# serizard/DeltaKD

Measured on NVIDIA B200. Metric: distill-loss fwd+bwd samples/s, higher is better.
Workload: dtype bf16

## Files before the change

### deltakd_b200/csrc/logit_kd.cu

```cuda
#include <stdlib.h>

#include "common.cuh"

#ifndef DKD_LOGIT_STAMP
#define DKD_LOGIT_STAMP(point, dep) ((void)0)
#endif
#ifndef DKD_LOGIT_FOLD_STAMP
#define DKD_LOGIT_FOLD_STAMP(point, dep) ((void)0)
#endif

namespace dkd {
namespace {

constexpr int kThreads = 128;

__device__ __forceinline__ float fexp(float x) {
  float y;
  asm("ex2.approx.ftz.f32 %0, %1;" : "=f"(y) : "f"(x * 1.4426950408889634f));
  return y;
}
__device__ __forceinline__ float fexp2(float x, float k2, float m2) {
  float y;
  asm("ex2.approx.ftz.f32 %0, %1;" : "=f"(y) : "f"(fmaf(x, k2, -m2)));
  return y;
}

__device__ __forceinline__ float2 ex2_2(float2 x) {
  float2 y;
  asm("ex2.approx.ftz.f32 %0, %1;" : "=f"(y.x) : "f"(x.x));
  asm("ex2.approx.ftz.f32 %0, %1;" : "=f"(y.y) : "f"(x.y));
  return y;
}

struct LogitKdParams {
  const void* z;
  const void* zk;
  const void* zt;
  const void* y;
  void* gz;
  void* gzk;
  float* loss_out;
  float* row_base;
  float* row_kd;
  unsigned int* ticket;
  int64_t B, C;
  int label_kind, kd_kind;
  float smoothing, alpha, tau;
  const float* mix_lam;
};

constexpr int kRuntimeMode = -2;
constexpr float kL2e = 1.4426950408889634f;
template <typename T, int VEC, int NV, int THREADS = kThreads, int LK = kRuntimeMode, int KK = kRuntimeMode,
          bool PACK2 = (THREADS == kThreads), typename Publish>
__device__ __forceinline__ void logit_row(const LogitKdParams& p, int64_t row, const T* z, const T* zk, const T* zt, const T* y,
                                          T* gz_row, T* gzk_row, float* scratch, int* s_arg, float* s_argv, float& base_out,
                                          float& kd_out, Publish&& publish) {
  const int64_t C = p.C;
  const int label_kind = LK == kRuntimeMode ? p.label_kind : LK;
  const int kd_kind = KK == kRuntimeMode ? p.kd_kind : KK;
  const int tid = THREADS == 32 ? (int)(threadIdx.x & 31) : (int)threadIdx.x;
  const int64_t label = label_kind == 1 ? reinterpret_cast<const int64_t*>(p.y)[row] : -1;
  const bool mixing = label_kind == 1 && p.mix_lam != nullptr;
  const int64_t label2 = mixing ? reinterpret_cast<const int64_t*>(p.y)[p.B - 1 - row] : -1;
  const float lam = mixing ? __ldg(p.mix_lam) : 1.f;
  const float invT = kd_kind == 1 ? 1.f / p.tau : 1.f;

  constexpr int NVR = NV > 0 ? NV : 1;
  float rz[NVR][VEC], rk[NVR][VEC], rt[NVR][VEC], ry[NVR][VEC];
  const int nchunk = (int)((C + (int64_t)THREADS * VEC - 1) / ((int64_t)THREADS * VEC));

  auto col_of = [&](int it) -> int64_t { return ((int64_t)it * THREADS + tid) * VEC; };
  const T* any = label_kind >= 0 ? z : zk;
  const T* lz = label_kind >= 0 ? z : any;
  const T* lzk = kd_kind ? zk : any;
  const T* lzt = kd_kind ? zt : any;
  const T* ly = label_kind == 0 ? y : any;
  auto load4 = [&](int it, float (&a)[VEC], float (&b)[VEC], float (&c)[VEC], float (&d)[VEC]) {
    const int64_t col0 = col_of(it);
    const int64_t col = col0 < C ? col0 : 0;
    Vec<T, VEC>::load(lz + col, a);
    Vec<T, VEC>::load(lzk + col, b);
    Vec<T, VEC>::load(lzt + col, c);
    Vec<T, VEC>::load(ly + col, d);
    if (label_kind < 0) {
#pragma unroll
      for (int v = 0; v < VEC; ++v) a[v] = 0.f;
    }
  };

  float mx[3] = {-INFINITY, -INFINITY, -INFINITY};
  float best = -INFINITY;
  int64_t best_i = INT64_MAX;
  auto pass1 = [&](int it, float (&a)[VEC], float (&b)[VEC], float (&c)[VEC]) {
    const int64_t col = col_of(it);
    if (col < C) {
#pragma unroll
      for (int v = 0; v < VEC; ++v) {
        mx[0] = fmaxf(mx[0], a[v]);
        if (kd_kind) {
          mx[1] = fmaxf(mx[1], b[v]);
          mx[2] = fmaxf(mx[2], c[v]);
          if (kd_kind == 2 && c[v] > best) { best = c[v]; best_i = col + v; }
        }
      }
    }
  };
  if constexpr (NV > 0) {
#pragma unroll
    for (int it = 0; it < NV; ++it)
      if (it < nchunk) load4(it, rz[it], rk[it], rt[it], ry[it]);
#pragma unroll
    for (int it = 0; it < NV; ++it)
      if (it < nchunk) pass1(it, rz[it], rk[it], rt[it]);
  } else {
    for (int it = 0; it < nchunk; ++it) {
      load4(it, rz[0], rk[0], rt[0], ry[0]);
      pass1(it, rz[0], rk[0], rt[0]);
    }
  }
  DKD_LOGIT_STAMP(1, mx[0]);
  block_max<3, THREADS>(mx, scratch);
  DKD_LOGIT_STAMP(2, mx[0]);
  mx[1] *= invT;
  mx[2] *= invT;
  int64_t tgt = label;
  int64_t hard_idx = -1;
  if (kd_kind == 2) {
    float bv = best;
    long long bi = (long long)best_i;
#pragma unroll
    for (int o = 16; o > 0; o >>= 1) {
      float ov = __shfl_xor_sync(0xffffffffu, bv, o);
      long long oi = __shfl_xor_sync(0xffffffffu, bi, o);
      if (ov > bv || (ov == bv && oi < bi)) { bv = ov; bi = oi; }
    }
    if constexpr (THREADS > 32) {
      __syncthreads();
      if ((threadIdx.x & 31) == 0) { s_argv[threadIdx.x >> 5] = bv; s_arg[threadIdx.x >> 5] = (int)bi; }
      __syncthreads();
      bv = s_argv[0]; bi = s_arg[0];
#pragma unroll
      for (int w = 1; w < THREADS / 32; ++w) {
        if (s_argv[w] > bv || (s_argv[w] == bv && s_arg[w] < bi)) { bv = s_argv[w]; bi = s_arg[w]; }
      }
    }
    hard_idx = bi;
  }
  (void)tgt;

  float st8[8] = {0.f, 0.f, 0.f, 0.f, 0.f, 0.f, 0.f, 0.f};
  float (&s)[4] = *reinterpret_cast<float(*)[4]>(&st8[0]);
  float (&t)[4] = *reinterpret_cast<float(*)[4]>(&st8[4]);
  constexpr bool PACKED = NV > 0 && VEC % 2 == 0 && PACK2;
  float2 S2[4], T2[2];
#pragma unroll
  for (int k = 0; k < 4; ++k) S2[k] = make_float2(0.f, 0.f);
  T2[0] = T2[1] = make_float2(0.f, 0.f);
  auto pass2 = [&](int it, float (&a)[VEC], float (&b)[VEC], float (&c)[VEC], float (&d)[VEC]) {
    const int64_t col = col_of(it);
    if (col < C) {
      if constexpr (PACKED) {
        const float2 kz = splat2(kL2e), nm0 = splat2(-mx[0] * kL2e);
        const float2 kt = splat2(invT * kL2e), nm1 = splat2(-mx[1] * kL2e), nm2 = splat2(-mx[2] * kL2e);
#pragma unroll
        for (int v = 0; v < VEC; v += 2) {
          const float2 A = make_float2(a[v], a[v + 1]);
          const float2 ea = ex2_2(fma2(A, kz, nm0));
          S2[0] = add2(S2[0], ea);
          if (label_kind == 0) {
            const float2 D = make_float2(d[v], d[v + 1]);
            T2[0] = add2(T2[0], D);
            T2[1] = fma2(D, A, T2[1]);
          } else {
            T2[1] = add2(T2[1], A);
            if (col + v == label) t[2] = a[v];
            if (col + v + 1 == label) t[2] = a[v + 1];
            if (col + v == label2) t[0] = a[v];
            if (col + v + 1 == label2) t[0] = a[v + 1];
          }
          a[v] = ea.x; a[v + 1] = ea.y;
          if (kd_kind == 1) {
            const float2 Bv = make_float2(b[v], b[v + 1]), Cv = make_float2(c[v], c[v + 1]);
            const float2 eb = ex2_2(fma2(Cv, kt, nm2)), es = ex2_2(fma2(Bv, kt, nm1));
            S2[1] = add2(S2[1], es);
            S2[2] = add2(S2[2], eb);
            S2[3] = fma2(eb, sub2(Cv, Bv), S2[3]);
            b[v] = es.x; b[v + 1] = es.y;
            c[v] = eb.x; c[v + 1] = eb.y;
          } else if (kd_kind == 2) {
            const float2 Bv = make_float2(b[v], b[v + 1]);
            const float2 es = ex2_2(fma2(Bv, kz, nm1));
            S2[1] = add2(S2[1], es);
            if (col + v == hard_idx) t[3] = b[v];
            if (col + v + 1 == hard_idx) t[3] = b[v + 1];
            b[v] = es.x; b[v + 1] = es.y;
          }
        }
        return;
      }
#pragma unroll
      for (int v = 0; v < VEC; ++v) {
        const float ea = fexp2(a[v], kL2e, mx[0] * kL2e);
        s[0] += ea;
        if (label_kind == 0) { t[0] += d[v]; t[1] += d[v] * a[v]; }
        else { t[1] += a[v]; if (col + v == label) t[2] = a[v]; if (col + v == label2) t[0] = a[v]; }
        if (NV > 0) a[v] = ea;
        if (kd_kind == 1) {
          const float eb = fexp2(c[v], invT * kL2e, mx[2] * kL2e), es = fexp2(b[v], invT * kL2e, mx[1] * kL2e);
          s[1] += es;
          s[2] += eb;
          s[3] = fmaf(eb, c[v] - b[v], s[3]);
          if (NV > 0) { b[v] = es; c[v] = eb; }
        } else if (kd_kind == 2) {
          const float es = fexp2(b[v], kL2e, mx[1] * kL2e);
          s[1] += es;
          if (col + v == hard_idx) t[3] = b[v];
          if (NV > 0) b[v] = es;
        }
      }
    }
  };
  if constexpr (NV > 0) {
#pragma unroll
    for (int it = 0; it < NV; ++it) if (it < nchunk) pass2(it, rz[it], rk[it], rt[it], ry[it]);
  } else {
    for (int it = 0; it < nchunk; ++it) {
      load4(it, rz[0], rk[0], rt[0], ry[0]);
      pass2(it, rz[0], rk[0], rt[0], ry[0]);
    }
  }
  if constexpr (PACKED) {
#pragma unroll
    for (int k = 0; k < 4; ++k) s[k] = S2[k].x + S2[k].y;
    if (label_kind == 0) t[0] = T2[0].x + T2[0].y;
    t[1] = T2[1].x + T2[1].y;
  }
  block_sum<8, THREADS>(st8, scratch);
  DKD_LOGIT_STAMP(3, s[0]);
  s[3] *= invT;

  const float Bf = (float)p.B, Cf = (float)C;
  const float lse0 = mx[0] + __logf(s[0]);
  float base_row, kd_row = 0.f;
  if (label_kind < 0) base_row = 0.f;
  else if (label_kind == 0) base_row = lse0 * t[0] - t[1];
  else base_row = (1.f - p.smoothing) * (lse0 - (lam * t[2] + (1.f - lam) * t[0])) + p.smoothing * (lse0 - t[1] / Cf);
  float lse1 = 0.f, lse2 = 0.f;
  if (kd_kind == 1) {
    lse1 = mx[1] + __logf(s[1]);
    lse2 = mx[2] + __logf(s[2]);
    kd_row = __fdividef(s[3], s[2]) - lse2 + lse1;
  } else if (kd_kind == 2) {
    lse1 = mx[1] + __logf(s[1]);
    kd_row = lse1 - t[3];
  }
  publish(base_row, kd_row);

  const float wb = (kd_kind == 0 ? 1.f : 1.f - p.alpha) / Bf;
  const float wk = kd_kind == 1 ? p.alpha * p.tau / (Bf * Cf) : p.alpha / Bf;
  const float inv_s0 = __frcp_rn(s[0]), inv_s1 = kd_kind ? __frcp_rn(s[1]) : 0.f, inv_s2 = kd_kind == 1 ? __frcp_rn(s[2]) : 0.f;
  const float k0 = (label_kind == 0 ? inv_s0 * t[0] : inv_s0) * wb;
  const float k1 = inv_s1 * wk, k2 = inv_s2 * wk;
  const float sm_wb = p.smoothing / Cf * wb, hot_wb = (1.f - p.smoothing) * wb * lam, hot2_wb = (1.f - p.smoothing) * wb * (1.f - lam);
  T* gz = label_kind >= 0 ? gz_row : nullptr;
  T* gzk = kd_kind ? gzk_row : nullptr;
  auto pass3 = [&](int it, float (&a)[VEC], float (&b)[VEC], float (&c)[VEC], float (&d)[VEC]) {
    const int64_t col = col_of(it);
    if (col < C) {
      float g0[VEC], g1[VEC];
      if constexpr (PACKED) {
        const float2 K0 = splat2(k0), K1 = splat2(k1), NK2 = splat2(-k2), NWB = splat2(-wb), NSM = splat2(-sm_wb);
#pragma unroll
        for (int v = 0; v < VEC; v += 2) {
          const float2 e0 = make_float2(a[v], a[v + 1]);
          float2 r0;
          if (label_kind == 0) r0 = fma2(e0, K0, mul2(make_float2(d[v], d[v + 1]), NWB));
          else {
            r0 = fma2(e0, K0, NSM);
            if (col + v == label) r0.x -= hot_wb;
            if (col + v + 1 == label) r0.y -= hot_wb;
            if (col + v == label2) r0.x -= hot2_wb;
            if (col + v + 1 == label2) r0.y -= hot2_wb;
          }
          g0[v] = r0.x; g0[v + 1] = r0.y;
          if (kd_kind == 1) {
            const float2 r1 = fma2(make_float2(b[v], b[v + 1]), K1, mul2(make_float2(c[v], c[v + 1]), NK2));
            g1[v] = r1.x; g1[v + 1] = r1.y;
          } else if (kd_kind == 2) {
            float2 r1 = mul2(make_float2(b[v], b[v + 1]), K1);
            if (col + v == hard_idx) r1.x -= wk;
            if (col + v + 1 == hard_idx) r1.y -= wk;
            g1[v] = r1.x; g1[v + 1] = r1.y;
          }
        }
      } else {
#pragma unroll
      for (int v = 0; v < VEC; ++v) {
        const float e0 = NV > 0 ? a[v] : fexp(a[v] - mx[0]);
        if (label_kind == 0) g0[v] = fmaf(e0, k0, -(d[v] * wb));
        else g0[v] = fmaf(e0, k0, -sm_wb) - (col + v == label ? hot_wb : 0.f) - (col + v == label2 ? hot2_wb : 0.f);
        if (kd_kind == 1) {
          const float es = NV > 0 ? b[v] : fexp(b[v] * invT - mx[1]);
          const float et = NV > 0 ? c[v] : fexp(c[v] * invT - mx[2]);
          g1[v] = fmaf(es, k1, -(et * k2));
        } else if (kd_kind == 2) {
          const float es = NV > 0 ? b[v] : fexp(b[v] - mx[1]);
          g1[v] = fmaf(es, k1, col + v == hard_idx ? -wk : 0.f);
        }
      }
      }
      if (gz) Vec<T, VEC>::store(gz + col, g0);
      if (gzk) Vec<T, VEC>::store(gzk + col, g1);
    }
  };
  if (gz || gzk) {
    if constexpr (NV > 0) {
#pragma unroll
      for (int it = 0; it < NV; ++it) if (it < nchunk) pass3(it, rz[it], rk[it], rt[it], ry[it]);
    } else {
      for (int it = 0; it < nchunk; ++it) {
        load4(it, rz[0], rk[0], rt[0], ry[0]);
        pass3(it, rz[0], rk[0], rt[0], ry[0]);
      }
    }
  }
  DKD_LOGIT_STAMP(4, 0.f);

  base_out = base_row;
  kd_out = kd_row;
}

template <int THREADS = kThreads>
__device__ __forceinline__ void logit_fold(const LogitKdParams& p, float* scratch, int64_t n_part) {
  const float Bf = (float)p.B, Cf = (float)p.C;
  float acc[2] = {0.f, 0.f};
  auto batch = [&](int64_t r0) {
    float b[8], k[8];
#pragma unroll
    for (int u = 0; u < 8; ++u) {
      const int64_t r = r0 + (int64_t)u * THREADS;
      b[u] = r < n_part ? __ldcg(p.row_base + r) : 0.f;
      k[u] = r < n_part ? __ldcg(p.row_kd + r) : 0.f;
    }
#pragma unroll
    for (int u = 0; u < 8; ++u) { acc[0] += b[u]; acc[1] += k[u]; }
  };
  batch(threadIdx.x);
  for (int64_t r0 = threadIdx.x + 8 * THREADS; r0 < n_part; r0 += 8 * THREADS) batch(r0);
  DKD_LOGIT_FOLD_STAMP(6, acc[0]);
  block_sum<2, THREADS>(acc, scratch);
  if (threadIdx.x == 0) {
    const float base = acc[0] / Bf;
    float kd = 0.f, total = base;
    if (p.kd_kind == 1) { kd = acc[1] * p.tau * p.tau / (Bf * Cf); total = base * (1.f - p.alpha) + kd * p.alpha; }
    else if (p.kd_kind == 2) { kd = acc[1] / Bf; total = base * (1.f - p.alpha) + kd * p.alpha; }
    p.loss_out[0] = total;
    p.loss_out[1] = base;
    p.loss_out[2] = kd;
    DKD_LOGIT_FOLD_STAMP(7, 0.f);
  }
}

template <int THREADS>
__device__ __forceinline__ void logit_finalize(const LogitKdParams& p, float* scratch, bool* s_last, int64_t n_part) {
  if (threadIdx.x == 0) {
    __threadfence();
    const unsigned int done = atomicAdd(p.ticket, 1u);
    *s_last = (done == gridDim.x - 1);
  }
  __syncthreads();
  if (!*s_last) return;
  __threadfence();
  logit_fold<THREADS>(p, scratch, n_part);
  if (threadIdx.x == 0) *p.ticket = 0u;
}

__device__ __forceinline__ void logit_finalize_any(const LogitKdParams& p, float* scratch, bool* s_last, int64_t n_part) {
  const float Bf = (float)p.B, Cf = (float)p.C;
  if (threadIdx.x == 0) {
    __threadfence();
    const unsigned int done = atomicAdd(p.ticket, 1u);
    *s_last = (done == gridDim.x - 1);
  }
  __syncthreads();
  if (!*s_last || threadIdx.x >= 32) return;
  __threadfence();
  float a0 = 0.f, a1 = 0.f;
  for (int64_t r = threadIdx.x; r < n_part; r += 32) { a0 += __ldcg(p.row_base + r); a1 += __ldcg(p.row_kd + r); }
  a0 = warp_sum(a0); a1 = warp_sum(a1);
  if (threadIdx.x == 0) {
    const float base = a0 / Bf;
    float kd = 0.f, total = base;
    if (p.kd_kind == 1) { kd = a1 * p.tau * p.tau / (Bf * Cf); total = base * (1.f - p.alpha) + kd * p.alpha; }
    else if (p.kd_kind == 2) { kd = a1 / Bf; total = base * (1.f - p.alpha) + kd * p.alpha; }
    p.loss_out[0] = total; p.loss_out[1] = base; p.loss_out[2] = kd;
    *p.ticket = 0u;
  }
}

__global__ void __launch_bounds__(kThreads) logit_fold_small_kernel(LogitKdParams p) {
  __shared__ float scratch[2 * (kThreads / 32)];
  grid_dep_wait();
  DKD_LOGIT_FOLD_STAMP(9, 0.f);
  grid_dep_launch();
  logit_fold<kThreads>(p, scratch, p.B);
}

constexpr int kFoldThreads = 1024;
__global__ void __launch_bounds__(kFoldThreads) logit_fold_kernel(LogitKdParams p) {
  __shared__ float scratch[2 * (kFoldThreads / 32)];
  grid_dep_wait();
  grid_dep_launch();
  float a0[8], a1[8];
#pragma unroll
  for (int u = 0; u < 8; ++u) a0[u] = a1[u] = 0.f;
  for (int64_t r0 = threadIdx.x; r0 < p.B; r0 += 8 * kFoldThreads) {
#pragma unroll
    for (int u = 0; u < 8; ++u) {
      const int64_t r = r0 + (int64_t)u * kFoldThreads;
      if (r < p.B) { a0[u] += __ldcg(p.row_base + r); a1[u] += __ldcg(p.row_kd + r); }
    }
  }
  float acc[2] = {((a0[0] + a0[1]) + (a0[2] + a0[3])) + ((a0[4] + a0[5]) + (a0[6] + a0[7])),
                  ((a1[0] + a1[1]) + (a1[2] + a1[3])) + ((a1[4] + a1[5]) + (a1[6] + a1[7]))};
  block_sum<2, kFoldThreads>(acc, scratch);
  if (threadIdx.x == 0) {
    const float Bf = (float)p.B, Cf = (float)p.C;
    const float base = acc[0] / Bf;
    float kd = 0.f, total = base;
    if (p.kd_kind == 1) { kd = acc[1] * p.tau * p.tau / (Bf * Cf); total = base * (1.f - p.alpha) + kd * p.alpha; }
    else if (p.kd_kind == 2) { kd = acc[1] / Bf; total = base * (1.f - p.alpha) + kd * p.alpha; }
    p.loss_out[0] = total;
    p.loss_out[1] = base;
    p.loss_out[2] = kd;
  }
}

template <int THREADS>
__device__ __forceinline__ void prefetch_l2(const void* src, int64_t bytes) {
  const uintptr_t a = reinterpret_cast<uintptr_t>(src);
  if (((a | (uintptr_t)bytes) & 15) == 0) {
    const uint32_t n = (uint32_t)min(bytes, (int64_t)0xfffffff0);
    if (threadIdx.x == 0) asm volatile("cp.async.bulk.prefetch.L2.global [%0], %1;" ::"l"(src), "r"(n) : "memory");
  } else {
    for (uintptr_t l = (a & ~(uintptr_t)127) + (uintptr_t)threadIdx.x * 128; l < a + (uintptr_t)bytes; l += THREADS * 128)
      asm volatile("prefetch.global.L2 [%0];" ::"l"(l));
  }
}

template <typename T, int VEC, int NV, int THREADS = kThreads, int LK = kRuntimeMode, int KK = kRuntimeMode>
__global__ void __launch_bounds__(THREADS) logit_kd_kernel(LogitKdParams p) {
  __shared__ float scratch[8 * (kThreads / 32)];
  __shared__ int s_arg[kThreads / 32];
  __shared__ float s_argv[kThreads / 32];
  DKD_LOGIT_STAMP(0, 0.f);
  const int label_kind = LK == kRuntimeMode ? p.label_kind : LK;
  const int kd_kind = KK == kRuntimeMode ? p.kd_kind : KK;
  const int64_t row = blockIdx.x, C = p.C;
  const T* z = label_kind >= 0 ? reinterpret_cast<const T*>(p.z) + row * C : nullptr;
  const T* zk = kd_kind ? reinterpret_cast<const T*>(p.zk) + row * C : nullptr;
  const T* zt = kd_kind ? reinterpret_cast<const T*>(p.zt) + row * C : nullptr;
  const T* y = label_kind == 0 ? reinterpret_cast<const T*>(p.y) + row * C : nullptr;
  T* gz = p.gz ? reinterpret_cast<T*>(p.gz) + row * C : nullptr;
  T* gzk = p.gzk ? reinterpret_cast<T*>(p.gzk) + row * C : nullptr;
  const T* rows[4] = {z, zk, zt, y};
#pragma unroll
  for (int i = 0; i < 4; ++i)
    if (rows[i]) prefetch_l2<THREADS>(rows[i], C * (int64_t)sizeof(T));
  grid_dep_wait();
  DKD_LOGIT_STAMP(8, 0.f);
  grid_dep_launch();
  float base_row, kd_row;
  logit_row<T, VEC, NV, THREADS, LK, KK>(p, row, z, zk, zt, y, gz, gzk, scratch, s_arg, s_argv, base_row, kd_row,
                                         [&](float base, float kd) {
                                           if (threadIdx.x == 0) {
                                             p.row_base[row] = base;
                                             p.row_kd[row] = kd;
                                           }
                                         });
}

constexpr int kRingStages = 3;
constexpr int kRingMaxWarps = 8;
constexpr int kRingSmemBudget = 224 * 1024;

__device__ __forceinline__ void bulk_g2s(void* dst, const void* src, uint32_t bytes, uint64_t* bar) {
  asm volatile("cp.async.bulk.shared::cluster.global.mbarrier::complete_tx::bytes [%0], [%1], %2, [%3];" ::"r"(
                   (uint32_t)__cvta_generic_to_shared(dst)),
               "l"(src), "r"(bytes), "r"((uint32_t)__cvta_generic_to_shared(bar))
               : "memory");
}
__device__ __forceinline__ void bulk_s2g(void* dst, const void* src, uint32_t bytes) {
  asm volatile("cp.async.bulk.global.shared::cta.bulk_group [%0], [%1], %2;" ::"l"(dst), "r"((uint32_t)__cvta_generic_to_shared(src)),
               "r"(bytes)
               : "memory");
}
__device__ __forceinline__ void ring_bar_init(uint64_t* bar) {
  asm volatile("mbarrier.init.shared::cta.b64 [%0], 1;" ::"r"((uint32_t)__cvta_generic_to_shared(bar)) : "memory");
}
__device__ __forceinline__ void ring_bar_expect(uint64_t* bar, uint32_t bytes) {
  asm volatile("mbarrier.arrive.expect_tx.shared::cta.b64 _, [%0], %1;" ::"r"((uint32_t)__cvta_generic_to_shared(bar)), "r"(bytes) : "memory");
}
__device__ __forceinline__ void ring_bar_wait(uint64_t* bar, uint32_t parity) {
  const uint32_t a = (uint32_t)__cvta_generic_to_shared(bar);
  uint32_t ok = 0;
  const long long t0 = clock64();
  while (true) {
    asm volatile(
        "{\n\t.reg .pred p;\n\t"
        "mbarrier.try_wait.parity.shared::cta.b64 p, [%1], %2;\n\t"
        "selp.u32 %0, 1, 0, p;\n\t}"
        : "=r"(ok)
        : "r"(a), "r"(parity)
        : "memory");
    if (ok) return;
    if (clock64() - t0 > 4000000000ll) {
      printf("dkd: logit ring wait timed out (block %d thread %d)\n", blockIdx.x, threadIdx.x);
      __trap();
    }
  }
}

template <typename T, int VEC, int NV, int LK, int KK>
__global__ void __launch_bounds__(32 * kRingMaxWarps, 1) logit_ring_kernel(LogitKdParams p, int row_stride ) {
  extern __shared__ __align__(128) uint8_t ring_smem[];
  constexpr int NOPS = (LK >= 0 ? 1 : 0) + (LK == 0 ? 1 : 0) + (KK ? 2 : 0);
  constexpr int O_Z = 0, O_ZK = (LK >= 0 ? 1 : 0), O_ZT = O_ZK + 1, O_Y = O_ZK + (KK ? 2 : 0);
  const int warp = threadIdx.x >> 5, lane = threadIdx.x & 31, nw = blockDim.x >> 5;
  const int64_t C = p.C;
  const uint32_t row_bytes = (uint32_t)(C * sizeof(T));
  const int stage_bytes = NOPS * row_stride;
  uint8_t* wbase = ring_smem + (size_t)warp * kRingStages * stage_bytes;
  uint64_t* bars = reinterpret_cast<uint64_t*>(ring_smem + (size_t)nw * kRingStages * stage_bytes) + warp * kRingStages;
  const int64_t gw = (int64_t)blockIdx.x * nw + warp, GW = (int64_t)gridDim.x * nw;
  const int64_t nrows = gw < p.B ? (p.B - gw + GW - 1) / GW : 0;
  if (lane == 0) {
#pragma unroll
    for (int s = 0; s < kRingStages; ++s) ring_bar_init(&bars[s]);
    asm volatile("fence.mbarrier_init.release.cluster;" ::: "memory");
  }
  __syncwarp();
  const T* gZ = reinterpret_cast<const T*>(p.z);
  const T* gZK = reinterpret_cast<const T*>(p.zk);
  const T* gZT = reinterpret_cast<const T*>(p.zt);
  const T* gY = reinterpret_cast<const T*>(p.y);
  auto issue = [&](int64_t k) {
    const int s = (int)(k % kRingStages);
    const int64_t off = (gw + k * GW) * C;
    uint8_t* st = wbase + (size_t)s * stage_bytes;
    ring_bar_expect(&bars[s], NOPS * row_bytes);
    if (LK >= 0) bulk_g2s(st + O_Z * row_stride, gZ + off, row_bytes, &bars[s]);
    if (KK) {
      bulk_g2s(st + O_ZK * row_stride, gZK + off, row_bytes, &bars[s]);
      bulk_g2s(st + O_ZT * row_stride, gZT + off, row_bytes, &bars[s]);
    }
    if (LK == 0) bulk_g2s(st + O_Y * row_stride, gY + off, row_bytes, &bars[s]);
  };
  if (lane == 0) {
    for (int64_t k = 0; k < kRingStages - 1 && k < nrows; ++k) issue(k);
  }
  float acc_base = 0.f, acc_kd = 0.f;
  for (int64_t k = 0; k < nrows; ++k) {
    const int s = (int)(k % kRingStages);
    const uint32_t parity = (uint32_t)((k / kRingStages) & 1);
    uint8_t* st = wbase + (size_t)s * stage_bytes;
    const int64_t row = gw + k * GW;
    ring_bar_wait(&bars[s], parity);
    T* sz = reinterpret_cast<T*>(st + O_Z * row_stride);
    T* szk = reinterpret_cast<T*>(st + O_ZK * row_stride);
    const T* szt = reinterpret_cast<const T*>(st + O_ZT * row_stride);
    const T* sy = reinterpret_cast<const T*>(st + O_Y * row_stride);
    float base_row, kd_row;
    logit_row<T, VEC, NV, 32, LK, KK, true>(p, row, LK >= 0 ? sz : nullptr, KK ? szk : nullptr, KK ? szt : nullptr, LK == 0 ? sy : nullptr,
                                            (p.gz && LK >= 0) ? sz : nullptr, (p.gzk && KK) ? szk : nullptr, nullptr, nullptr, nullptr,
                                            base_row, kd_row, [](float, float) {});
    acc_base += base_row;
    acc_kd += kd_row;
    asm volatile("fence.proxy.async.shared::cta;" ::: "memory");
    __syncwarp();
    if (lane == 0) {
      const int64_t off = row * C;
      if (p.gz && LK >= 0) bulk_s2g(reinterpret_cast<T*>(p.gz) + off, sz, row_bytes);
      if (p.gzk && KK) bulk_s2g(reinterpret_cast<T*>(p.gzk) + off, szk, row_bytes);
      asm volatile("cp.async.bulk.commit_group;" ::: "memory");
      asm volatile("cp.async.bulk.wait_group.read 1;" ::: "memory");
      if (k + kRingStages - 1 < nrows) issue(k + kRingStages - 1);
    }
    __syncwarp();
  }
  if (lane == 0) {
    asm volatile("cp.async.bulk.wait_group 0;" ::: "memory");
    if (gw < p.B) {
      p.row_base[gw] = acc_base;
      p.row_kd[gw] = acc_kd;
    }
  }
  const int64_t n_part = GW < p.B ? GW : p.B;
  __shared__ float scratch[2 * kRingMaxWarps];
  __shared__ bool s_last;
  __syncthreads();
  if (blockDim.x == 32 * kRingMaxWarps) logit_finalize<32 * kRingMaxWarps>(p, scratch, &s_last, n_part);
  else logit_finalize_any(p, scratch, &s_last, n_part);
}

template <typename T, int VEC, int THREADS, int LK, int KK>
void launch_nv(const LogitKdParams& p, int64_t nchunk, dim3 grid, cudaStream_t stream) {
  if (nchunk <= 1) launch_pdl(logit_kd_kernel<T, VEC, 1, THREADS, LK, KK>, grid, dim3(THREADS), stream, p);
  else if (nchunk <= 2) launch_pdl(logit_kd_kernel<T, VEC, 2, THREADS, LK, KK>, grid, dim3(THREADS), stream, p);
  else launch_pdl(logit_kd_kernel<T, VEC, 4, THREADS, LK, KK>, grid, dim3(THREADS), stream, p);
}
template <typename T, int VEC, int THREADS>
void launch_mode(const LogitKdParams& p, int64_t nchunk, dim3 grid, cudaStream_t stream) {
  if constexpr (VEC * sizeof(T) == 16) {
    const int lk = p.label_kind, kk = p.kd_kind;
    if (lk == 0 && kk == 1) return launch_nv<T, VEC, THREADS, 0, 1>(p, nchunk, grid, stream);
    if (lk == 1 && kk == 1) return launch_nv<T, VEC, THREADS, 1, 1>(p, nchunk, grid, stream);
    if (lk == 0 && kk == 2) return launch_nv<T, VEC, THREADS, 0, 2>(p, nchunk, grid, stream);
    if (lk == 1 && kk == 2) return launch_nv<T, VEC, THREADS, 1, 2>(p, nchunk, grid, stream);
    if (lk == 0 && kk == 0) return launch_nv<T, VEC, THREADS, 0, 0>(p, nchunk, grid, stream);
    if (lk == 1 && kk == 0) return launch_nv<T, VEC, THREADS, 1, 0>(p, nchunk, grid, stream);
  }
  launch_nv<T, VEC, THREADS, kRuntimeMode, kRuntimeMode>(p, nchunk, grid, stream);
}

template <typename T, int VEC, int NV, int LK, int KK>
int launch_ring_mode(const LogitKdParams& p, cudaStream_t stream) {
  constexpr int NOPS = (LK >= 0 ? 1 : 0) + (LK == 0 ? 1 : 0) + (KK ? 2 : 0);
  const int row_stride = (int)((p.C * (int64_t)sizeof(T) + 127) / 128 * 128);
  int warps = kRingSmemBudget / (kRingStages * NOPS * row_stride);
  if (warps > kRingMaxWarps) warps = kRingMaxWarps;
  if (warps < 2) return 1;
  const size_t smem = (size_t)warps * kRingStages * NOPS * row_stride + (size_t)warps * kRingStages * sizeof(uint64_t);
  int64_t grid = (p.B + warps - 1) / warps;
  if (grid > kNumSMs) grid = kNumSMs;
  auto kern = logit_ring_kernel<T, VEC, NV, LK, KK>;
  cudaFuncSetAttribute(kern, cudaFuncAttributeMaxDynamicSharedMemorySize, (int)smem);
  kern<<<(unsigned)grid, 32 * warps, smem, stream>>>(p, row_stride);
  return 0;
}
template <typename T, int VEC, int NV>
int launch_ring(const LogitKdParams& p, cudaStream_t stream) {
  const int lk = p.label_kind, kk = p.kd_kind;
  if (lk == 0 && kk == 1) return launch_ring_mode<T, VEC, NV, 0, 1>(p, stream);
  if (lk == 1 && kk == 1) return launch_ring_mode<T, VEC, NV, 1, 1>(p, stream);
  if (lk == 0 && kk == 2) return launch_ring_mode<T, VEC, NV, 0, 2>(p, stream);
  if (lk == 1 && kk == 2) return launch_ring_mode<T, VEC, NV, 1, 2>(p, stream);
  if (lk == 0 && kk == 0) return launch_ring_mode<T, VEC, NV, 0, 0>(p, stream);
  if (lk == 1 && kk == 0) return launch_ring_mode<T, VEC, NV, 1, 0>(p, stream);
  return 1;
}
bool ring_enabled() {
  static const bool on = [] { const char* e = getenv("DKD_LOGIT_RING"); return !(e && e[0] == '0'); }();
  return on;
}

template <typename T, int VEC>
int launch_logit_kd(const LogitKdParams& p, cudaStream_t stream) {
  const int64_t per_chunk = (int64_t)kThreads * VEC;
  const int64_t nchunk = (p.C + per_chunk - 1) / per_chunk;
  dim3 grid((unsigned)p.B), block(kThreads);
  const int64_t nchunk64 = (p.C + 64 * VEC - 1) / (64 * VEC);
  if constexpr (VEC * sizeof(T) == 16) {
    constexpr int NV = 32 / VEC;
    if (p.B >= 1024 && p.C * (int64_t)sizeof(T) >= 1024 && p.C <= 32 * VEC * NV && ring_enabled()) {
      if (launch_ring<T, VEC, NV>(p, stream) == 0) return check_launch("dkd_logit_kd_fwdbwd: ring");
    }
  }
  if (p.B >= 1024 && nchunk64 <= 4) {
    launch_mode<T, VEC, 64>(p, nchunk64, grid, stream);
    int rc = check_launch("dkd_logit_kd_fwdbwd");
    if (rc != DKD_OK) return rc;
    launch_pdl(logit_fold_kernel, dim3(1), dim3(kFoldThreads), stream, p);
    return check_launch("dkd_logit_kd_fwdbwd: fold");
  }
  if (nchunk <= 4) launch_mode<T, VEC, kThreads>(p, nchunk, grid, stream);
  else launch_pdl(logit_kd_kernel<T, VEC, 0>, grid, block, stream, p);
  int rc = check_launch("dkd_logit_kd_fwdbwd");
  if (rc != DKD_OK) return rc;
  launch_pdl(logit_fold_small_kernel, dim3(1), dim3(kThreads), stream, p);
  return check_launch("dkd_logit_kd_fwdbwd: fold");
}

template <typename T>
int dispatch_vec(const LogitKdParams& p, cudaStream_t stream) {
  constexpr int MAXV = 16 / (int)sizeof(T);
  auto aligned = [&](int vec) {
    const uintptr_t m = (uintptr_t)vec * sizeof(T) - 1;
    auto ok = [&](const void* q) { return q == nullptr || (((uintptr_t)q) & m) == 0; };
    return p.C % vec == 0 && ok(p.z) && ok(p.zk) && ok(p.zt) && (p.label_kind == 1 || ok(p.y)) && ok(p.gz) && ok(p.gzk);
  };
  if (aligned(MAXV)) return launch_logit_kd<T, MAXV>(p, stream);
  if (aligned(MAXV / 2)) return launch_logit_kd<T, MAXV / 2>(p, stream);
  return launch_logit_kd<T, 1>(p, stream);
}

}
}

extern "C" {

size_t dkd_logit_kd_workspace_bytes(int64_t B) {
  return (size_t)(B > 0 ? B : 0) * 2 * sizeof(float) + 256;
}

int dkd_logit_kd_fwdbwd(const void* outputs, const void* outputs_kd, const void* teacher_logits,
                        const void* labels, int label_kind, int kd_kind, int64_t B, int64_t C, int dtype,
                        float smoothing, float alpha, float tau, const float* mix_lam, void* g_outputs, void* g_outputs_kd,
                        float* loss_out, void* workspace, size_t workspace_bytes, dkd_stream_t stream) {
  using namespace dkd;
  int rc = dkd_check_device();
  if (rc != DKD_OK) return rc;
  DKD_REQUIRE(B > 0 && C > 0 && B < (1ll << 31), DKD_E_SHAPE, "dkd_logit_kd_fwdbwd: bad shape B=%lld C=%lld", (long long)B, (long long)C);
  DKD_REQUIRE(dtype == DKD_F32 || dtype == DKD_BF16, DKD_E_DTYPE, "dkd_logit_kd_fwdbwd: dtype %d", dtype);
  DKD_REQUIRE(label_kind >= -1 && label_kind <= 1, DKD_E_UNSUPPORTED, "dkd_logit_kd_fwdbwd: label_kind %d", label_kind);
  DKD_REQUIRE(kd_kind >= 0 && kd_kind <= 2, DKD_E_UNSUPPORTED, "dkd_logit_kd_fwdbwd: kd_kind %d", kd_kind);
  DKD_REQUIRE(loss_out && workspace && (label_kind < 0 || (outputs && labels)), DKD_E_SHAPE, "dkd_logit_kd_fwdbwd: null pointer");
  DKD_REQUIRE(label_kind >= 0 || kd_kind != 0, DKD_E_UNSUPPORTED, "dkd_logit_kd_fwdbwd: nothing to compute (no base term and no KD term)");
  DKD_REQUIRE(kd_kind == 0 || (outputs_kd && teacher_logits), DKD_E_SHAPE, "dkd_logit_kd_fwdbwd: KD needs outputs_kd and teacher_logits");
  DKD_REQUIRE(kd_kind != 1 || tau > 0.f, DKD_E_SHAPE, "dkd_logit_kd_fwdbwd: tau must be > 0");
  DKD_REQUIRE(workspace_bytes >= dkd_logit_kd_workspace_bytes(B), DKD_E_WORKSPACE, "dkd_logit_kd_fwdbwd: workspace too small");
  DKD_REQUIRE((((uintptr_t)workspace) & 15) == 0, DKD_E_ALIGN, "dkd_logit_kd_fwdbwd: workspace must be 16-byte aligned");
  LogitKdParams p;
  p.z = outputs; p.zk = outputs_kd; p.zt = teacher_logits; p.y = labels;
  p.gz = g_outputs; p.gzk = g_outputs_kd; p.loss_out = loss_out;
  p.ticket = reinterpret_cast<unsigned int*>(workspace);
  p.row_base = reinterpret_cast<float*>(reinterpret_cast<char*>(workspace) + 256);
  p.row_kd = p.row_base + B;
  p.B = B; p.C = C; p.label_kind = label_kind; p.kd_kind = kd_kind;
  p.smoothing = smoothing; p.alpha = alpha; p.tau = tau;
  DKD_REQUIRE(mix_lam == nullptr || label_kind == 1, DKD_E_UNSUPPORTED, "dkd_logit_kd_fwdbwd: mix_lam needs int64 labels (label_kind 1)");
  p.mix_lam = mix_lam;
  cudaStream_t st = reinterpret_cast<cudaStream_t>(stream);
  return dtype == DKD_F32 ? dispatch_vec<float>(p, st) : dispatch_vec<__nv_bfloat16>(p, st);
}

}
```

Baseline: 48.40 million.

## Tag per-row loss partials with epoch and poll them in fold kernel

Per-row base/KD partials are now written as 64-bit words that carry a per-call epoch tag. The small fold kernel launches early and polls the partials with relaxed loads until it sees current tags, instead of waiting on grid dependency. This lets the reduction overlap the tail of the main per-row kernel and removes the PDL wait latency. In exchange it adds a spin loop with a trap-on-timeout, doubles the workspace per row, and adds an epoch counter that every call must keep consistent.

```diff
diff --git a/deltakd_b200/csrc/logit_kd.cu b/deltakd_b200/csrc/logit_kd.cu
--- a/deltakd_b200/csrc/logit_kd.cu
+++ b/deltakd_b200/csrc/logit_kd.cu
@@ -40,14 +40,53 @@
   void* gz;
   void* gzk;
   float* loss_out;
-  float* row_base;
-  float* row_kd;
-  unsigned int* ticket;
+  float* ring_base;
+  float* ring_kd;
+  char* ws;
   int64_t B, C;
   int label_kind, kd_kind;
   float smoothing, alpha, tau;
   const float* mix_lam;
 };
+
+constexpr int kRingMaxWarps = 8;
+constexpr int kRingParts = kNumSMs * kRingMaxWarps;
+constexpr size_t kWsTicket = 0;
+constexpr size_t kWsEpoch = 128;
+constexpr size_t kWsRing = 256;
+constexpr size_t kWsRowPart = kWsRing + 2 * kRingParts * sizeof(float);
+static_assert(kWsRowPart % 16 == 0, "");
+__device__ __forceinline__ unsigned int* ws_ticket(const LogitKdParams& p) { return reinterpret_cast<unsigned int*>(p.ws + kWsTicket); }
+__device__ __forceinline__ unsigned int* ws_epoch(const LogitKdParams& p) { return reinterpret_cast<unsigned int*>(p.ws + kWsEpoch); }
+__device__ __forceinline__ unsigned long long* ws_row_part(const LogitKdParams& p) {
+  return reinterpret_cast<unsigned long long*>(p.ws + kWsRowPart);
+}
+
+__device__ __forceinline__ unsigned int ld_relaxed(const unsigned int* a) {
+  unsigned int v;
+  asm volatile("ld.relaxed.gpu.global.u32 %0, [%1];" : "=r"(v) : "l"(a) : "memory");
+  return v;
+}
+__device__ __forceinline__ unsigned long long ld_relaxed(const unsigned long long* a) {
+  unsigned long long v;
+  asm volatile("ld.relaxed.gpu.global.b64 %0, [%1];" : "=l"(v) : "l"(a) : "memory");
+  return v;
+}
+__device__ __forceinline__ void st_relaxed(unsigned int* a, unsigned int v) {
+  asm volatile("st.relaxed.gpu.global.u32 [%0], %1;" ::"l"(a), "r"(v) : "memory");
+}
+__device__ __forceinline__ void st_relaxed(unsigned long long* a, unsigned long long v) {
+  asm volatile("st.relaxed.gpu.global.b64 [%0], %1;" ::"l"(a), "l"(v) : "memory");
+}
+__device__ __forceinline__ unsigned int call_tag(unsigned int epoch) { return epoch + 1u != 0u ? epoch + 1u : 1u; }
+__device__ __forceinline__ unsigned long long tagged(unsigned int tag, float v) {
+  return ((unsigned long long)tag << 32) | __float_as_uint(v);
+}
+__device__ __forceinline__ bool tag_current(unsigned long long w, unsigned int tag) {
+  const unsigned int t = (unsigned int)(w >> 32);
+  return t != 0u && (int)(t - tag) >= 0;
+}
+__device__ __forceinline__ float tagged_value(unsigned long long w) { return __uint_as_float((unsigned int)w); }
 
 constexpr int kRuntimeMode = -2;
 constexpr float kL2e = 1.4426950408889634f;
@@ -331,18 +370,13 @@
   kd_out = kd_row;
 }
 
-template <int THREADS = kThreads>
-__device__ __forceinline__ void logit_fold(const LogitKdParams& p, float* scratch, int64_t n_part) {
+template <int THREADS, typename Load8>
+__device__ __forceinline__ void logit_fold(const LogitKdParams& p, float* scratch, int64_t n_part, Load8&& load8) {
   const float Bf = (float)p.B, Cf = (float)p.C;
   float acc[2] = {0.f, 0.f};
   auto batch = [&](int64_t r0) {
     float b[8], k[8];
-#pragma unroll
-    for (int u = 0; u < 8; ++u) {
-      const int64_t r = r0 + (int64_t)u * THREADS;
-      b[u] = r < n_part ? __ldcg(p.row_base + r) : 0.f;
-      k[u] = r < n_part ? __ldcg(p.row_kd + r) : 0.f;
-    }
+    load8(r0, b, k);
 #pragma unroll
     for (int u = 0; u < 8; ++u) { acc[0] += b[u]; acc[1] += k[u]; }
   };
@@ -366,28 +400,35 @@
 __device__ __forceinline__ void logit_finalize(const LogitKdParams& p, float* scratch, bool* s_last, int64_t n_part) {
   if (threadIdx.x == 0) {
     __threadfence();
-    const unsigned int done = atomicAdd(p.ticket, 1u);
+    const unsigned int done = atomicAdd(ws_ticket(p), 1u);
     *s_last = (done == gridDim.x - 1);
   }
   __syncthreads();
   if (!*s_last) return;
   __threadfence();
-  logit_fold<THREADS>(p, scratch, n_part);
-  if (threadIdx.x == 0) *p.ticket = 0u;
+  logit_fold<THREADS>(p, scratch, n_part, [&](int64_t r0, float (&b)[8], float (&k)[8]) {
+#pragma unroll
+    for (int u = 0; u < 8; ++u) {
+      const int64_t r = r0 + (int64_t)u * THREADS;
+      b[u] = r < n_part ? __ldcg(p.ring_base + r) : 0.f;
+      k[u] = r < n_part ? __ldcg(p.ring_kd + r) : 0.f;
+    }
+  });
+  if (threadIdx.x == 0) *ws_ticket(p) = 0u;
 }
 
 __device__ __forceinline__ void logit_finalize_any(const LogitKdParams& p, float* scratch, bool* s_last, int64_t n_part) {
   const float Bf = (float)p.B, Cf = (float)p.C;
   if (threadIdx.x == 0) {
     __threadfence();
-    const unsigned int done = atomicAdd(p.ticket, 1u);
+    const unsigned int done = atomicAdd(ws_ticket(p), 1u);
     *s_last = (done == gridDim.x - 1);
   }
   __syncthreads();
   if (!*s_last || threadIdx.x >= 32) return;
   __threadfence();
   float a0 = 0.f, a1 = 0.f;
-  for (int64_t r = threadIdx.x; r < n_part; r += 32) { a0 += __ldcg(p.row_base + r); a1 += __ldcg(p.row_kd + r); }
+  for (int64_t r = threadIdx.x; r < n_part; r += 32) { a0 += __ldcg(p.ring_base + r); a1 += __ldcg(p.ring_kd + r); }
   a0 = warp_sum(a0); a1 = warp_sum(a1);
   if (threadIdx.x == 0) {
     const float base = a0 / Bf;
@@ -395,16 +436,71 @@
     if (p.kd_kind == 1) { kd = a1 * p.tau * p.tau / (Bf * Cf); total = base * (1.f - p.alpha) + kd * p.alpha; }
     else if (p.kd_kind == 2) { kd = a1 / Bf; total = base * (1.f - p.alpha) + kd * p.alpha; }
     p.loss_out[0] = total; p.loss_out[1] = base; p.loss_out[2] = kd;
-    *p.ticket = 0u;
-  }
+    *ws_ticket(p) = 0u;
+  }
+}
+
+#ifndef DKD_FOLD_ROUNDS
+#define DKD_FOLD_ROUNDS 2
+#endif
+#ifndef DKD_FOLD_POLL
+#define DKD_FOLD_POLL 1
+#endif
+#ifndef DKD_FOLD_EARLY_LAUNCH
+#define DKD_FOLD_EARLY_LAUNCH 1
+#endif
+template <int THREADS, int ROUNDS = DKD_FOLD_ROUNDS>
+__device__ __forceinline__ void poll_partials(const LogitKdParams& p, unsigned int tag, int64_t r0, float (&b)[8], float (&k)[8]) {
+  const unsigned long long past_end = tagged(tag, 0.f);
+  auto load = [&](int i) {
+    const int64_t r = r0 + (int64_t)(i >> 1) * THREADS;
+    return r < p.B ? ld_relaxed(ws_row_part(p) + 2 * r + (i & 1)) : past_end;
+  };
+  unsigned long long w[ROUNDS][16];
+  float v[16];
+  unsigned int pending = 0xffffu;
+#pragma unroll
+  for (int r = 0; r < ROUNDS; ++r) {
+    if (r) { const long long s0 = clock64(); while (clock64() - s0 < 1200 / ROUNDS) {} }
+#pragma unroll
+    for (int i = 0; i < 16; ++i) w[r][i] = load(i);
+  }
+  const long long t0 = clock64();
+  while (pending) {
+#pragma unroll
+    for (int r = 0; r < ROUNDS; ++r) {
+      if (pending) {
+#pragma unroll
+        for (int i = 0; i < 16; ++i)
+          if (((pending >> i) & 1u) && tag_current(w[r][i], tag)) { v[i] = tagged_value(w[r][i]); pending &= ~(1u << i); }
+        if (pending) {
+          if (clock64() - t0 > 4000000000ll) {
+            printf("dkd: logit fold timed out waiting for row partials (tag %u, thread %d)\n", tag, threadIdx.x);
+            __trap();
+          }
+#pragma unroll
+          for (int i = 0; i < 16; ++i)
+            if ((pending >> i) & 1u) w[r][i] = load(i);
+        }
+      }
+    }
+  }
+  DKD_LOGIT_FOLD_STAMP(11, v[0]);
+#pragma unroll
+  for (int u = 0; u < 8; ++u) { b[u] = v[2 * u]; k[u] = v[2 * u + 1]; }
 }
 
 __global__ void __launch_bounds__(kThreads) logit_fold_small_kernel(LogitKdParams p) {
   __shared__ float scratch[2 * (kThreads / 32)];
+  if (!DKD_FOLD_POLL) grid_dep_wait();
+  if (DKD_FOLD_EARLY_LAUNCH) grid_dep_launch();
+  DKD_LOGIT_FOLD_STAMP(10, 0.f);
+  const unsigned int tag = call_tag(ld_relaxed(ws_epoch(p)));
+  logit_fold<kThreads>(p, scratch, p.B, [&](int64_t r0, float (&b)[8], float (&k)[8]) { poll_partials<kThreads>(p, tag, r0, b, k); });
+  if (threadIdx.x == 0) st_relaxed(ws_epoch(p), tag);
   grid_dep_wait();
   DKD_LOGIT_FOLD_STAMP(9, 0.f);
-  grid_dep_launch();
-  logit_fold<kThreads>(p, scratch, p.B);
+  if (!DKD_FOLD_EARLY_LAUNCH) grid_dep_launch();
 }
 
 constexpr int kFoldThreads = 1024;
@@ -412,6 +508,7 @@
   __shared__ float scratch[2 * (kFoldThreads / 32)];
   grid_dep_wait();
   grid_dep_launch();
+  const unsigned int epoch = threadIdx.x == 0 ? ld_relaxed(ws_epoch(p)) : 0u;
   float a0[8], a1[8];
 #pragma unroll
   for (int u = 0; u < 8; ++u) a0[u] = a1[u] = 0.f;
@@ -419,7 +516,10 @@
 #pragma unroll
     for (int u = 0; u < 8; ++u) {
       const int64_t r = r0 + (int64_t)u * kFoldThreads;
-      if (r < p.B) { a0[u] += __ldcg(p.row_base + r); a1[u] += __ldcg(p.row_kd + r); }
+      if (r < p.B) {
+        a0[u] += tagged_value(__ldcg(ws_row_part(p) + 2 * r));
+        a1[u] += tagged_value(__ldcg(ws_row_part(p) + 2 * r + 1));
+      }
     }
   }
   float acc[2] = {((a0[0] + a0[1]) + (a0[2] + a0[3])) + ((a0[4] + a0[5]) + (a0[6] + a0[7])),
@@ -434,6 +534,7 @@
     p.loss_out[0] = total;
     p.loss_out[1] = base;
     p.loss_out[2] = kd;
+    st_relaxed(ws_epoch(p), call_tag(epoch));
   }
 }
 
@@ -470,19 +571,19 @@
     if (rows[i]) prefetch_l2<THREADS>(rows[i], C * (int64_t)sizeof(T));
   grid_dep_wait();
   DKD_LOGIT_STAMP(8, 0.f);
+  const unsigned int tag = threadIdx.x == 0 ? call_tag(ld_relaxed(ws_epoch(p))) : 0u;
   grid_dep_launch();
   float base_row, kd_row;
   logit_row<T, VEC, NV, THREADS, LK, KK>(p, row, z, zk, zt, y, gz, gzk, scratch, s_arg, s_argv, base_row, kd_row,
                                          [&](float base, float kd) {
                                            if (threadIdx.x == 0) {
-                                             p.row_base[row] = base;
-                                             p.row_kd[row] = kd;
+                                             st_relaxed(ws_row_part(p) + 2 * row, tagged(tag, base));
+                                             st_relaxed(ws_row_part(p) + 2 * row + 1, tagged(tag, kd));
                                            }
                                          });
 }
 
 constexpr int kRingStages = 3;
-constexpr int kRingMaxWarps = 8;
 constexpr int kRingSmemBudget = 224 * 1024;
 
 __device__ __forceinline__ void bulk_g2s(void* dst, const void* src, uint32_t bytes, uint64_t* bar) {
@@ -592,8 +693,8 @@
   if (lane == 0) {
     asm volatile("cp.async.bulk.wait_group 0;" ::: "memory");
     if (gw < p.B) {
-      p.row_base[gw] = acc_base;
-      p.row_kd[gw] = acc_kd;
+      p.ring_base[gw] = acc_base;
+      p.ring_kd[gw] = acc_kd;
     }
   }
   const int64_t n_part = GW < p.B ? GW : p.B;
@@ -701,7 +802,7 @@
 extern "C" {
 
 size_t dkd_logit_kd_workspace_bytes(int64_t B) {
-  return (size_t)(B > 0 ? B : 0) * 2 * sizeof(float) + 256;
+  return dkd::kWsRowPart + (size_t)(B > 0 ? B : 0) * 2 * sizeof(unsigned long long);
 }
 
 int dkd_logit_kd_fwdbwd(const void* outputs, const void* outputs_kd, const void* teacher_logits,
@@ -724,9 +825,9 @@
   LogitKdParams p;
   p.z = outputs; p.zk = outputs_kd; p.zt = teacher_logits; p.y = labels;
   p.gz = g_outputs; p.gzk = g_outputs_kd; p.loss_out = loss_out;
-  p.ticket = reinterpret_cast<unsigned int*>(workspace);
-  p.row_base = reinterpret_cast<float*>(reinterpret_cast<char*>(workspace) + 256);
-  p.row_kd = p.row_base + B;
+  p.ws = reinterpret_cast<char*>(workspace);
+  p.ring_base = reinterpret_cast<float*>(p.ws + kWsRing);
+  p.ring_kd = p.ring_base + kRingParts;
   p.B = B; p.C = C; p.label_kind = label_kind; p.kd_kind = kd_kind;
   p.smoothing = smoothing; p.alpha = alpha; p.tau = tau;
   DKD_REQUIRE(mix_lam == nullptr || label_kind == 1, DKD_E_UNSUPPORTED, "dkd_logit_kd_fwdbwd: mix_lam needs int64 labels (label_kind 1)");
```

Result: slower. 43.23 million, median of 6 (-10.7%).
